# lesterphillip/SVCC23_FastSVC

Hardware: AMD Instinct MI355X
Metric: audio samples/sec (24 kHz) FastSVC generator fwd (higher is better)
Workload: dtype bf16 (bf16 MFMA products, f32 accumulate; bf16 storage); 1 GPU; cfg3: 64 x 10 s utterances per GPU, F=1500 frames, T=240000 samples, generator fastsvc.yaml (144->[192,96,48,24], x[2,4,4,5]), spk_emb on; global_batch=64, utterance_samples=240000, parallelism=utterance-parallel x1

## Files before the change

### include/fastsvc_hip.h

```cpp
#ifndef FASTSVC_HIP_H
#define FASTSVC_HIP_H

#include <stddef.h>
#include <stdint.h>

#ifdef __cplusplus
extern "C" {
#endif

#define FASTSVC_ABI_VERSION 1
#define FASTSVC_MAX_STAGES 8

enum {
    FASTSVC_OK = 0,
    FASTSVC_E_INVALID = -1,
    FASTSVC_E_MISSING = -2,
    FASTSVC_E_WORKSPACE = -3,
    FASTSVC_E_HIP = -4,
    FASTSVC_E_UNSUPPORTED = -5
};

typedef struct fastsvc_config {
    int32_t in_channels;
    int32_t n_stages;
// ... 46 lines not shown
                            float* out, int32_t B, int32_t F, const int32_t* lengths,
                            const int32_t* group, const int32_t* own_lo, const int32_t* own_hi,
                            void* workspace, size_t workspace_bytes,
                            void* scratch, size_t scratch_bytes, void* stream);

int fastsvc_norm_group_stats(const void* u, int32_t storage, int32_t B, int32_t C, int32_t ld, const int32_t* lengths,
                             int32_t len_mul, const int32_t* group, const int32_t* own_lo, const int32_t* own_hi,
                             double* stats_out, void* scratch, size_t scratch_bytes, void* stream);

int fastsvc_stream_prepare(void* stream);

int fastsvc_stream_release(void* stream);

void fastsvc_split_half(const float* x, int64_t n, uint16_t* f16_hi, uint16_t* f16_lo, uint16_t* bf16);

int fastsvc_workspace_tap(const fastsvc_plan* plan, int32_t B, int32_t F, const char* tap_name,
                          size_t* byte_offset, int64_t* numel, int64_t shape3[3]);

int fastsvc_autotune(const fastsvc_plan* plan, const void* dev_blob,
                     const float* ppg, const float* sine, const float* lft, const float* spk_emb,
                     float* out, int32_t B, int32_t F,
                     void* workspace, size_t workspace_bytes, void* stream, int32_t* n_trials);

int fastsvc_tuned_count(const fastsvc_plan* plan);
int fastsvc_tuned_get(const fastsvc_plan* plan, int32_t index, char* key_out, int32_t shape_out[5]);
int fastsvc_tuned_set(const fastsvc_plan* plan, const char* key, const int32_t shape[5]);

typedef struct fastsvc_launch_record {
    char layer[64];
    char kernel[40];
    double flops;
    double bytes;
    float ms;
} fastsvc_launch_record;

int fastsvc_forward_profile(const fastsvc_plan* plan, const void* dev_blob,
                            const float* ppg, const float* sine, const float* lft, const float* spk_emb,
                            float* out, int32_t B, int32_t F, const int32_t* lengths,
                            void* workspace, size_t workspace_bytes, void* stream,
                            fastsvc_launch_record* records, int32_t max_records, int32_t* n_records);

int fastsvc_forward_launch_count(const fastsvc_plan* plan, int32_t with_spk_emb);
double fastsvc_flops_per_sample(const fastsvc_plan* plan);

size_t fastsvc_signal_scratch_bytes(int32_t B, int32_t F);
int fastsvc_signal_generate(const float* f0, float* out, void* scratch, int32_t B, int32_t F, int32_t hop,
                            float sample_rate, float sine_amp, float noise_amp,
                            const int32_t* types, int32_t ntypes, uint64_t seed, void* stream);

int fastsvc_gather_padded(const float* const* src, const int32_t* lens, const int32_t* pitches, float* dst,
                          int32_t B, int32_t C, int32_t width, void* stream);

int fastsvc_gather_time_major(const float* packed, int64_t packed_elems, const int64_t* offsets, const int32_t* lens,
                              float* dst, int32_t B, int32_t C, int32_t width, void* stream);

int fastsvc_pcm16_pack(const float* y, const int32_t* lens, const int64_t* offsets, int16_t* dst, int64_t dst_elems,
                       int32_t B, int32_t width, void* stream);

typedef struct fastsvc_row_report {
    int32_t nonfinite;
    int32_t clipped;
    float   max_abs;
    int32_t reserved;
} fastsvc_row_report;

int fastsvc_pcm16_pack_checked(const float* y, const int32_t* lens, const int64_t* offsets, int16_t* dst, int64_t dst_elems,
// ... 80 lines not shown
```

### svcc23_fastsvc_amd/csrc/fastsvc_hx.hip

```cpp
#include "fastsvc_kernels.h"

namespace fastsvc {
#ifdef FASTSVC_ACT_2B
namespace FASTSVC_ACT_NS {
#endif

#include "fastsvc_device.inc"

#include "fastsvc_hx_common.inc"

template <int MW, int NW, bool RELOAD, bool OPT_LAST = false, int NS = 3 * MW * HX_NP, int SOFF = 0, bool ADV = true, bool HOLD = false>
__device__ __forceinline__ void hx_unit_direct(f32x4 (&acc)[NW][MW], const unsigned char* tile, const int (&aoff)[3],
                                               int lo_off, HxWeightStream<NS>& ws, bool do_last = true, bool hold = false) {
    constexpr int NSTEP = 3 * NW;
    constexpr int PF = HX_NP == 1 ? (MW >= 3 ? 2 : 3) : 1;
    HxFrag a[PF + 1];
    #pragma unroll
    for (int q = 0; q < PF && q < NSTEP; ++q) a[q] = hx_read(tile, aoff[q / NW] + (q % NW) * 16 * HX_ROW, lo_off);
    #pragma unroll
    for (int s = 0; s < NSTEP; ++s) {
        const int tap = s / NW, n = s % NW;
        if (s + PF < NSTEP) {
            a[(s + PF) % (PF + 1)] = hx_read(tile, aoff[(s + PF) / NW] + ((s + PF) % NW) * 16 * HX_ROW, lo_off);
            __builtin_amdgcn_sched_barrier(0);
// ... 426 lines not shown
    const __amdgpu_buffer_rsrc_t yr = make_rsrc(p.last_y + (long)b * p.last_y_b, p.ldy);
    #pragma unroll
    for (int n = 0; n < NW; ++n) {
        f32x4 s = acc[n][0] * kw[0];
        #pragma unroll
        for (int m = 1; m < MW; ++m) s += acc[n][m] * kw[m];
        #pragma unroll
        for (int e = 0; e < 4; ++e) {
            float v = s[e];
            v += __builtin_bit_cast(float, __builtin_amdgcn_mov_dpp(__builtin_bit_cast(int, v), 0xB1, 0xF, 0xF, true));
            v += __builtin_bit_cast(float, __builtin_amdgcn_mov_dpp(__builtin_bit_cast(int, v), 0x4E, 0xF, 0xF, true));
            v += __builtin_bit_cast(float, __builtin_amdgcn_mov_dpp(__builtin_bit_cast(int, v), 0x141, 0xF, 0xF, true));
            v += __builtin_bit_cast(float, __builtin_amdgcn_mov_dpp(__builtin_bit_cast(int, v), 0x140, 0xF, 0xF, true));
            s[e] = v;
        }
        const int t = PAIRS ? tcol0 + (n >> 1) * 32 + (lane >> 4) * 8 + (n & 1) * 4 : tcol0 + n * 16 + (lane >> 4) * 4;
        buf_store4(yr, ((lane & 15) == 0 && t < p.T) ? t * 4 : OOB_OFF, s + bias);
    }
}

#ifndef FASTSVC_HX_W8
#define FASTSVC_HX_W8 1
#endif
constexpr bool hx_w8(int MODE, bool tailk, int S) {
    return FASTSVC_HX_W8 != 0 && HX_NP == 1 && !tailk && (MODE == MODE_DIRECT || MODE == MODE_POLY || (MODE == MODE_DEC2 && S == 2));
}
#ifndef FASTSVC_HX_CARRY
#define FASTSVC_HX_CARRY 1
#endif
constexpr bool hx_carry(int MODE, bool tailk, int S, int NT) {
    return FASTSVC_HX_CARRY != 0 && hx_w8(MODE, tailk, S) && MODE == MODE_DIRECT && S == 1 && NT == 128;
}

template <int MW, int NW, int WM, int WN, int MODE, int EPI, int S, bool WSTATIC, bool TAILK = false>
__global__ __launch_bounds__(512, (hx_min_waves<MW, NW, MODE, EPI, S, TAILK>()))
void conv_hx_kernel(const ConvParams p0) {
    constexpr bool UPH = MODE == MODE_UPHEAD;
    constexpr bool POLY = MODE == MODE_POLY, DEC2 = MODE == MODE_DEC2, CHAIN = MODE == MODE_CHAIN || MODE == MODE_CHAIN1 || UPH;
    constexpr bool IN1 = MODE == MODE_CHAIN1;
    constexpr bool WLB = MODE == MODE_CHAIN && S == 2;
    constexpr bool XR = MODE == MODE_DIRECT && S > 1;
    constexpr int NT = 16 * NW * WN;
    constexpr int NTV = CHAIN ? NT + 16 : NT;
    constexpr int HB = CHAIN ? 4 : 0;
    constexpr int NPROD_T = 256;
    constexpr bool W8 = hx_w8(MODE, TAILK, S);
    constexpr int SPARE = W8 ? 8 : 4;
    constexpr int MAXW = NTV + (MODE == MODE_DIRECT ? (W8 ? 64 : 56) : (W8 ? 16 : 8));
    constexpr int ITEMS = (MAXW + NPROD_T - 1) / NPROD_T;
    constexpr int NWS = DEC2 ? 4 : 3;
    constexpr int NVAR = DEC2 ? 2 : 1;
    constexpr int NSLOT = NWS * MW * HX_NP;
    constexpr bool TRACKS = AMAX_TRACK && ((CHAIN && MODE != MODE_UPHEAD) || (MODE == MODE_DIRECT && (EPI == EPI_RES || EPI == EPI_RANK1)));
    extern __shared__ __attribute__((aligned(16))) unsigned char smem_raw[];

    const int tid = threadIdx.x;
    const int lane = tid & 63;
    const int wave = __builtin_amdgcn_readfirstlane(tid >> 6);
    const bool producer = wave >= 4;
    const int cw = wave & 3;
    const int wave_m = cw / WN;
    const int wave_n = cw - wave_m * WN;
    const int z = blockIdx.z;
    const int sig = z / p0.B;
    const int b = z - sig * p0.B;
    ConvParams p = p0;
    if (p0.lens) {
        const int frames = p0.lens[b];
        p.T = frames * p0.len_mul;
        p.x_T = frames * p0.xlen_mul;
    }
    const int mg = blockIdx.y * WM + wave_m;
    const bool active = !producer && mg < p.ngroups;
    const int halo = (MODE == MODE_DIRECT || CHAIN) ? p.dil : 1;
// ... 1 lines not shown
    const int W = NTV + 2 * halo_al;
    const int nch = p.nch32;
    const int CINp = nch * HX_KC;
    const int flags = p.flags;
    const int ntx = (p.T + NT - 1) / NT;
    const int tile0 = blockIdx.x * p.tpw;
    const int ntiles = min(p.tpw, ntx - tile0);
    if (ntiles <= 0) return;
    const int nunits = ntiles * (XR ? 2 * nch : nch);
#ifdef FASTSVC_TIMELINE
    const int wg_lin = blockIdx.x + gridDim.x * (blockIdx.y + gridDim.y * blockIdx.z);
    unsigned long long* tlw = (p.tl && wg_lin < p.tl_wgs) ? p.tl + ((long)wg_lin * 8 + wave) * 64 : nullptr;
    int tli = 0;
    auto stamp = [&](int tag) {
        if (tlw && lane == 0 && tli < 62) { tlw[tli++] = ((unsigned long long)tag << 56) | (__builtin_readcyclecounter() & 0x00ffffffffffffffull); }
    };
    stamp(1);
    if (tlw && lane == 0) {
        tlw[62] = __builtin_amdgcn_s_getreg(4 | (0 << 6) | (31 << 11));
        tlw[63] = __builtin_amdgcn_s_getreg(20 | (0 << 6) | (31 << 11));
    }
#else
    auto stamp = [](int) {};
#endif

    if constexpr (hx_min_waves<MW, NW, MODE, EPI, S, TAILK>() >= 4) {
        const int wg_id = blockIdx.x + gridDim.x * (blockIdx.y + gridDim.y * blockIdx.z);
        if ((wg_id >> 8) & 1) {
            for (int k = 0; k < p.stagger; ++k) __builtin_amdgcn_s_sleep(16);
        }
    }
    double* sstat = reinterpret_cast<double*>(smem_raw);
    float2* ncoef = reinterpret_cast<float2*>(smem_raw + sizeof(double) * 2 * 16 * MW * WM);
    unsigned char* tiles = reinterpret_cast<unsigned char*>(ncoef + CINp + 8);
    __shared__ unsigned s_amax, s_cnt;
    __shared__ float s_inv[HX_NP == 2 ? 2 * 16 * MW * WM : 4];
    __shared__ __attribute__((aligned(16))) float s_mid[CHAIN ? 2 * (16 * MW * WM + 32) : 4];
    float sx = 1.f;
    float sx2 = 1.f;
    float s_mid_scale = 1.f;
    const int ninv = 16 * MW * p.ngroups;
    const float* invtab = (HX_NP == 2 && p.whx_inv) ? p.whx_inv + (long)sig * p.whx_inv_sig : nullptr;
    auto operand_scales = [&]() {
#ifndef FASTSVC_EXP_NOSCALE
        if constexpr (HX_NP == 2) {
            if (p.amax_in) {
                auto bound_of = [&](int entry, int s) -> float {
                    float bd = amax_read(p.amax_in, entry);
                    #pragma unroll
                    for (int j = 0; j < 2; ++j)
                        if (p.bnd_path[j]) { const float* q = p.bnd_path[j] + (long)s * p.bnd_sig[j]; bd = bd * q[0] + q[1]; }
                    return bd;
                };
                float bound = bound_of(sig * p.amax_in_sig + b, sig);
                if (p.amax_in2 > 0) bound = fmaxf(bound, bound_of(p.amax_in2 + b, 1));
                if (flags & F_PRE_NORM) bound += sqrtf((float)p.x_T);
                if constexpr (CHAIN) {
                    if (invtab) {
                        const float* cst = invtab + (UPH ? 3 : 2) * ninv;
                        if constexpr (IN1) bound = bound * cst[2] + cst[3];
                        s_mid_scale = hx_scale_for(bound * cst[0] + cst[1]);
                    }
                }
                sx = hx_scale_for(bound);
            }
            if constexpr (XR) {
                if (p.amax_x2) {
// ... 347 lines not shown
            if constexpr (XR) {
                const int tl = xc_tl;
                pos_next(xc_tl, xc_ch);
                const int t_start = (tile0 + tl) * NT - halo_al;
                const int g0 = (t_start + 8 * XROWS) / XROWS - 8;
                const int r0 = (g0 + xg) * XROWS - t_start;
                #pragma unroll
                for (int jj = 0; jj < XJ; ++jj) {
                    float px[XJ][8];
                    #pragma unroll
                    for (int c = 0; c < 8; ++c) px[jj][c] = act_unpack1(pw[jj][c]);
                    hx8 h;
                    #pragma unroll
                    for (int c = 0; c < 8; ++c) h[c] = (hx_t)(HX_NP == 2 ? px[jj][c] * sx2 : px[jj][c]);
                    typedef unsigned u32x4w __attribute__((ext_vector_type(4)));
                    u32x4w lp = {0u, 0u, 0u, 0u};
                    if constexpr (HX_NP == 2) {
                        const u32x4w hp = __builtin_bit_cast(u32x4w, h);
                        #pragma unroll
                        for (int k = 0; k < 4; ++k) lp[k] = hx_lo_pair(hp[k], px[jj][2 * k] * sx2, px[jj][2 * k + 1] * sx2);
                    }
                    #pragma unroll
                    for (int ph = 0; ph < S; ++ph) {
                        const int r = r0 + jj * S + ph;
                        const int off = hx_lds_off((unsigned)r < (unsigned)W ? r : W, xoct);
                        *reinterpret_cast<hx8*>(tile + off) = h;
                        if constexpr (HX_NP == 2) *reinterpret_cast<u32x4w*>(tile + lo_off + off) = lp;
                    }
                }
            }
        };
        if constexpr (XR) {
            pwin_t pa[ITEMS][8];
            act1_t xb[XJ][8];
            unsigned oka = 0;
            pload(0, pa, oka);
            ploadX(1, xb);
            stamp(2);
            setup_shared();
            pcommit(0, pa, oka, tiles);
            unsigned okn = 0;
            if constexpr (!WSTATIC) pload(2, pa, okn);
            stamp(3);
            __syncthreads();
            stamp(4);
            for (int u = 0; u < nunits; u += 2) {
                if constexpr (WSTATIC) pload(u + 2, pa, oka);
                pcommitX(u + 1, xb, tiles + bufsz);
                if constexpr (!WSTATIC) ploadX(u + 3, xb);
                stamp(5);
                __syncthreads();
                stamp(6);
                if constexpr (WSTATIC) ploadX(u + 3, xb); else oka = okn;
                pcommit(u + 2, pa, oka, tiles);
                if constexpr (!WSTATIC) pload(u + 4, pa, okn);
                stamp(5);
                __syncthreads();
                stamp(6);
            }
        } else {
        constexpr bool PSPLIT = POLY && hx_poly_staged<MW, NW, MODE, EPI, S>();
        EpiRsrc Rp;
        const bool pact = mg < p.ngroups;
        if constexpr (PSPLIT) {
            const long ct = (long)p.COUT * p.ldy;
            const float* nul = p.bias;
            Rp.y = act_rsrc(p.y ? p.y : nul, p.y ? (long)sig * p.y_sig + (long)b * p.y_b : 0, p.y ? ct : 0);
            const bool has_y2 = (flags & F_AFF_OUT) != 0;
            Rp.y2 = act_rsrc(has_y2 ? p.y2 : nul, has_y2 ? (long)sig * p.y2_sig + (long)b * p.y2_b : 0, has_y2 ? ct : 0);
            const bool has_ss = (flags & (F_STATS | F_AFF_OUT)) != 0;
            Rp.ss = act_rsrc(has_ss ? p.ss_out : nul, has_ss ? (long)b * p.ss_out_b : 0, has_ss ? 2 * ct : 0);
            Rp.res = Rp.y; Rp.r1x = Rp.y;
        }
        auto ppass2 = [&](int un) {
#ifdef FASTSVC_ACT_2B
            if constexpr (PSPLIT) {
                const int etl = e_tl, ech = e_ch;
                pos_next(e_tl, e_ch);
                if (un < nunits && ech == nch - 1) {
                    const int tcolw = (tile0 + etl) * NT + wave_n * (NW * 16);
                    const unsigned char* Pw = tiles + 2 * bufsz + cw * hx_poly_patch_bytes<MW, NW, S>();
                    HxPolyPass2<MW, NW, EPI, S, hx_poly_mc<MW>(), MW> P2;
                    float s1p[MW], s2p[MW];
                    #pragma unroll
                    for (int m = 0; m < MW; ++m) { s1p[m] = 0.f; s2p[m] = 0.f; }
                    if (pact) P2.request(p, Rp, mg, tcolw, lane);
                    __syncthreads();
                    if (pact) {
                        P2.run(p, Rp, Pw, s1p, s2p, mg, tcolw, lane);
                        if (flags & F_STATS) {
                            #pragma unroll
// ... 718 lines not shown
        }
#define FASTSVC_HXC(k) if (kind == k) return hx_launch_kind<MW, NW, WM, WN, MODE_CHAIN, k, 1>(grid, smem, stream, p);
        FASTSVC_HXC(EPI_PLAIN) FASTSVC_HXC(EPI_RES) FASTSVC_HXC(EPI_RANK1)
#undef FASTSVC_HXC
        return hipErrorInvalidValue;
    } else if constexpr (MODE == MODE_DEC2) {
        const size_t patch = hx_dec2_staged<MW, NW, MODE_DEC2>() ? 4 * (size_t)hx_dec2_patch_bytes<MW, NW>() : 0;
        if (p.s == 1 && (p.ldx & 3) == 0) return hx_launch_kind<MW, NW, WM, WN, MODE_DEC2, EPI_PLAIN, 2>(grid, smem + patch, stream, p);
        return hx_launch_kind<MW, NW, WM, WN, MODE_DEC2, EPI_PLAIN, 1>(grid, smem + patch, stream, p);
    } else if constexpr (MODE == MODE_POLY) {
#define FASTSVC_HXP(sv) \
        if (p.s == sv) return aff ? hx_launch_kind<MW, NW, WM, WN, MODE_POLY, EPI_AFF, sv>(grid, smem + (hx_poly_staged<MW, NW, MODE_POLY, EPI_AFF, sv>() ? 4 * hx_poly_patch_bytes<MW, NW, sv>() : 0), stream, p) \
                                  : hx_launch_kind<MW, NW, WM, WN, MODE_POLY, EPI_PLAIN, sv>(grid, smem + (hx_poly_staged<MW, NW, MODE_POLY, EPI_PLAIN, sv>() ? 4 * hx_poly_patch_bytes<MW, NW, sv>() : 0), stream, p);
        FASTSVC_HXP(2) FASTSVC_HXP(4) FASTSVC_HXP(5)
#undef FASTSVC_HXP
        return hipErrorInvalidValue;
    } else {
        const int kind = aff ? EPI_AFF : p.r1x ? EPI_RANK1 : p.res ? EPI_RES : EPI_PLAIN;
        size_t est = 0;
        constexpr bool PAIRS = hx_pairs_epi<MW, NW, MODE_DIRECT>();
        if ((kind == EPI_AFF && hx_estage<MW, NW, MODE_DIRECT, EPI_AFF>()) || (kind == EPI_RES && hx_estage<MW, NW, MODE_DIRECT, EPI_RES>()))
            est = sizeof(float) * 4 * (size_t)(aff ? (p.res ? 3 : 2) : 1) * (PAIRS ? MW * (NW / 2) * 256 : MW * NW * EST_ITEM_FLOATS);
        if (MW == 2 && p.nch32 == 1 && !p.x2 &&
            ((kind == EPI_AFF && hx_est2<MW, NW, MODE_DIRECT, EPI_AFF>()) || (kind == EPI_RES && hx_est2<MW, NW, MODE_DIRECT, EPI_RES>())))
            est *= 2;
        if (PAIRS) est += sizeof(float) * 4 * 16 * 36;
        if (kind == EPI_AFF && hx_two_cu<MW, NW, MODE_DIRECT, EPI_AFF>() && !(p.lens && (((p.len_mul | p.xlen_mul) & 3) != 0)))
            est += hx_gsum_bytes<MW>();
        if (p.x2) {
            if (kind != EPI_AFF || p.res || p.x2_T * p.s2 != p.T || (p.lens && (((p.len_mul | p.xlen_mul) & 3) != 0)))
                return hipErrorInvalidValue;
            if (w8 && p.s2 == 2 && W / p.s2 + 5 > 128) return hipErrorInvalidValue;
            if (w8 && !conv_hx_x2_rows_ok(p)) return hipErrorInvalidValue;
#define FASTSVC_HXX(sv, stat) if (p.s2 == sv) return hx_launch_instance<&conv_hx_kernel<MW, NW, WM, WN, MODE_DIRECT, EPI_AFF, sv, stat>>(grid, smem + est, stream, p);
            if constexpr (MW * NW <= 12) {
                if constexpr (MW == 2) { if (p.nch32 == 1) { FASTSVC_HXX(5, true) } }
                else { FASTSVC_HXX(2, false) FASTSVC_HXX(4, false) }
            }
#undef FASTSVC_HXX
            return hipErrorInvalidValue;
        }
#define FASTSVC_HX(k) if (kind == k) return hx_launch_kind<MW, NW, WM, WN, MODE_DIRECT, k, 1>(grid, smem + est, stream, p);
        FASTSVC_HX(EPI_PLAIN) FASTSVC_HX(EPI_RES) FASTSVC_HX(EPI_RANK1) FASTSVC_HX(EPI_AFF)
#undef FASTSVC_HX
        return hipErrorInvalidValue;
    }
}

hipError_t launch_conv_hx(const ConvParams& p, const ConvLaunch& cfg, hipStream_t stream) {
    if (p.ntaps != 3 || (p.T & 3) || !p.whx || p.nch32 * HX_KC > 512) return hipErrorInvalidValue;
#define FASTSVC_HXS(md, mw, nw, wm, wn) \
    if (cfg.MW == mw && cfg.NW == nw && cfg.WM == wm && cfg.WN == wn) \
        return hx_launch_shape<mw, nw, wm, wn, md>(p, cfg.nsig, stream);
    if (p.mode == MODE_DIRECT) {
        if (p.dil < 1 || p.dil > 28) return hipErrorInvalidValue;
        FASTSVC_HXS(MODE_DIRECT, 2, 2, 1, 4) FASTSVC_HXS(MODE_DIRECT, 2, 3, 1, 4)
        FASTSVC_HXS(MODE_DIRECT, 3, 2, 1, 4) FASTSVC_HXS(MODE_DIRECT, 3, 3, 1, 4)
        FASTSVC_HXS(MODE_DIRECT, 3, 4, 2, 2) FASTSVC_HXS(MODE_DIRECT, 3, 6, 2, 2)
        FASTSVC_HXS(MODE_DIRECT, 3, 8, 4, 1)
    } else if (p.mode == MODE_POLY) {
        if (p.dil != 1) return hipErrorInvalidValue;
        FASTSVC_HXS(MODE_POLY, 2, 2, 1, 4) FASTSVC_HXS(MODE_POLY, 2, 3, 1, 4)
        FASTSVC_HXS(MODE_POLY, 3, 2, 1, 4) FASTSVC_HXS(MODE_POLY, 3, 2, 2, 2)
    } else if (p.mode == MODE_CHAIN) {
        if (p.dil < 1 || p.dil > 4 || p.dil2 < 1 || p.dil2 > 4 || !p.bias_mid || p.CMID != p.COUT) return hipErrorInvalidValue;
        if (p.ngroups > cfg.WM) return hipErrorInvalidValue;
        FASTSVC_HXS(MODE_CHAIN, 2, 2, 1, 4) FASTSVC_HXS(MODE_CHAIN, 2, 3, 1, 4)
        FASTSVC_HXS(MODE_CHAIN, 3, 2, 1, 4) FASTSVC_HXS(MODE_CHAIN, 3, 3, 1, 4)
        FASTSVC_HXS(MODE_CHAIN, 3, 4, 2, 2) FASTSVC_HXS(MODE_CHAIN, 3, 6, 2, 2)
    } else if (p.mode == MODE_UPHEAD) {
        if (p.dil != 1 || p.dil2 != 1 || !p.bias_mid || p.CMID != p.COUT || p.ngroups > cfg.WM) return hipErrorInvalidValue;
        FASTSVC_HXS(MODE_UPHEAD, 3, 4, 4, 1) FASTSVC_HXS(MODE_UPHEAD, 3, 2, 2, 2)
        FASTSVC_HXS(MODE_UPHEAD, 3, 2, 1, 4) FASTSVC_HXS(MODE_UPHEAD, 2, 2, 1, 4)
    } else if (p.mode == MODE_CHAIN1) {
        if (p.dil < 1 || p.dil > 4 || p.dil2 < 1 || p.dil2 > 4 || !p.bias_mid || p.CMID != p.COUT || p.CIN > 32 ||
            !p.in1_w || !p.in1_b || p.ngroups > cfg.WM) return hipErrorInvalidValue;
        FASTSVC_HXS(MODE_CHAIN1, 2, 2, 1, 4) FASTSVC_HXS(MODE_CHAIN1, 2, 3, 1, 4)
    } else if (p.mode == MODE_DEC2) {
        if (p.dil != 1 || !p.bias2 || !p.y2) return hipErrorInvalidValue;
        FASTSVC_HXS(MODE_DEC2, 3, 2, 1, 4) FASTSVC_HXS(MODE_DEC2, 3, 3, 1, 4) FASTSVC_HXS(MODE_DEC2, 3, 2, 2, 2)
        FASTSVC_HXS(MODE_DEC2, 3, 4, 2, 2) FASTSVC_HXS(MODE_DEC2, 3, 4, 4, 1)
    }
#undef FASTSVC_HXS
    return hipErrorInvalidValue;
}

#ifndef FASTSVC_ACT_2B
bool conv_hx_x2_ok(int MW, int nch32, int s2) { return MW == 2 ? (nch32 == 1 && s2 == 5) : MW == 3 ? (s2 == 2 || s2 == 4) : false; }
bool conv_hx_x2_rows_ok(const ConvParams& p) { return p.s2 != 2 || ((p.lens ? p.x2len_mul : p.x2_T) & 3) == 0; }
bool conv_hx_tail_ok(int mode, int MW, int epi_kind, int S) { return hx_tail_instance(MW, mode, epi_kind, S); }

bool conv_hx_shape(int mode, int MW, int NW, int WM, int WN) {
    if (mode == MODE_POLY)
        return (MW == 2 && WM == 1 && WN == 4 && (NW == 2 || NW == 3)) ||
               (MW == 3 && NW == 2 && ((WM == 1 && WN == 4) || (WM == 2 && WN == 2)));
    if (mode == MODE_DEC2)
        return MW == 3 && ((WM == 1 && WN == 4 && (NW == 2 || NW == 3)) || (WM == 2 && WN == 2 && (NW == 2 || NW == 4)) ||
                           (WM == 4 && WN == 1 && NW == 4));
    if (mode == MODE_CHAIN1) return MW == 2 && WM == 1 && WN == 4 && (NW == 2 || NW == 3);
    if (mode == MODE_UPHEAD)
        return (MW == 3 && ((NW == 4 && WM == 4 && WN == 1) || (NW == 2 && WM == 2 && WN == 2) || (NW == 2 && WM == 1 && WN == 4))) ||
               (MW == 2 && NW == 2 && WM == 1 && WN == 4);
    if (mode == MODE_CHAIN)
        return (WM == 1 && WN == 4 && (MW == 2 || MW == 3) && (NW == 2 || NW == 3)) ||
               (MW == 3 && WM == 2 && WN == 2 && (NW == 4 || NW == 6));
    if (mode != MODE_DIRECT) return false;
    if (MW == 2) return WM == 1 && WN == 4 && (NW == 2 || NW == 3);
    if (MW != 3) return false;
    if (WM == 1 && WN == 4) return NW == 2 || NW == 3;
    if (WM == 2 && WN == 2) return NW == 4 || NW == 6;
    return WM == 4 && WN == 1 && NW == 8;
}
#endif

#ifdef FASTSVC_ACT_2B
}
#endif
}
```

### svcc23_fastsvc_amd/csrc/fastsvc_kernels.h

```cpp
#pragma once
#include <hip/hip_runtime.h>
#include <stdint.h>

#if defined(FASTSVC_ACT_BF16) && defined(FASTSVC_ACT_F16)
#error "FASTSVC_ACT_BF16 and FASTSVC_ACT_F16 exclude each other"
#endif
#if defined(FASTSVC_ACT_BF16)
#define FASTSVC_ACT_2B 1
#define FASTSVC_ACT_NS bf16
#elif defined(FASTSVC_ACT_F16)
#define FASTSVC_ACT_2B 1
#define FASTSVC_ACT_NS f16
#endif

namespace fastsvc {

enum : int {
    MODE_DIRECT = 0,
    MODE_DECIMATE = 1,
    MODE_STRETCH = 2,
    MODE_POLY = 3,
    MODE_WINO = 4,
    MODE_DEC2 = 5,
    MODE_CHAIN = 6,
    MODE_CHAIN1 = 7,
    MODE_UPHEAD = 8
};

enum : int {
    F_PRE_LRELU = 1,
    F_PRE_AFFINE = 2,
    F_PRE_NORM = 4,
    F_POST_LRELU = 8,
    F_STATS = 16,
    F_AFF_OUT = 32
};

constexpr float LRELU_SLOPE = 0.2f;
constexpr double IN_EPS = 1e-5;

struct ConvParams {
    const float* x;
    long x_sig, x_b;
    int x_T;
    int CIN, KC, nchunks;
    const float* w;
    long w_sig;
    const float* bias;
    long bias_sig;
    int Q;
    const void* whx;
    long whx_sig;
    int nch32;
    int stagger;
    const float* bias_mid;
    long bias_mid_sig;
    const float* last_w;
    const float* last_b;
    float* last_y;
    long last_y_b;
    int xsplit;
    const float* in1_w;
    const float* in1_b;
    long in1_w_sig, in1_b_sig;
    int CMID, nch32b, dil2;
    int ngroups;
    const float* whx_inv;
    long whx_inv_sig;
// ... 103 lines not shown
    long hd_sig, hd_b;
    int hd_ld, hd_s;
    int tpw;
    int small;
};

enum : int { DBG_NO_LOAD = 1, DBG_NO_MFMA = 2, DBG_NO_EPILOGUE = 4, DBG_NO_COMMIT = 8, DBG_NO_WEIGHTS = 16 };
#ifdef FASTSVC_DEBUG_SWITCHES
#define FASTSVC_DBG_ON(p, flag) (((p).dbg & (flag)) != 0)
#else
#define FASTSVC_DBG_ON(p, flag) false
#endif

struct ConvLaunch {
    int MW;
    int NW;
    int WM, WN;
    int nsig;
    int pipe;
};

bool conv_pipe_supported(const ConvParams& p);
bool conv_poly_shape(int MW, int NW, int WM, int WN);
int conv_ws_resident(int MW, int NW, int mode, int epi_kind);
bool conv_ws_tail_ok(int MW, int NW, int mode, int epi_kind, int S);

hipError_t launch_conv(const ConvParams& p, const ConvLaunch& cfg, hipStream_t stream);

hipError_t launch_conv_hx(const ConvParams& p, const ConvLaunch& cfg, hipStream_t stream);
bool conv_hx_shape(int mode, int MW, int NW, int WM, int WN);
bool conv_hx_tail_ok(int mode, int MW, int epi_kind, int S);
bool conv_hx_x2_ok(int MW, int nch32, int s2);
bool conv_hx_x2_rows_ok(const ConvParams& p);

hipError_t launch_conv_wx(const ConvParams& p, const ConvLaunch& cfg, hipStream_t stream);
bool conv_wx_shape(int mode, int MW, int NW, int WM, int WN);
bool conv_wx_fits(int nch32, int dil);
bool conv_wx_supported(const ConvParams& p);

hipError_t launch_in1_conv(const float* x, long x_sig, const float* w, const float* bias, long w_sig, long b_sig,
                           float* y, int nsig, int B, int C, int T, const int* lens, int len_mul, hipStream_t stream,
                           float* amax_out = nullptr);

hipError_t launch_noop(hipStream_t stream);
hipError_t launch_stats_exact(const float* u, double* st, int B, int C, int ld, const int* lens, int len_mul, int max_frames,
                              hipStream_t stream);
hipError_t launch_amax_inputs(const float* sig, long sig_stride, const float* ppg, int B, int C, int F, int hop,
                              const int* lens, float* amax_in, float* zero, int nzero, hipStream_t stream);

constexpr int NORMGROUP_CHUNK = 2048;
inline int norm_group_chunks(long ld) { return (int)((ld + NORMGROUP_CHUNK - 1) / NORMGROUP_CHUNK); }
hipError_t launch_norm_group_partials(const float* u, double* part, int B, int C, int ld, const int* lens, int len_mul,
                                      const int* group, const int* own_lo, const int* own_hi, hipStream_t stream);
hipError_t launch_norm_group_pool(const double* part, double* st, int B, int C, int ld, const int* lens, int len_mul,
                                  const int* group, const int* own_lo, const int* own_hi, float* amax_raise, hipStream_t stream);

hipError_t launch_pointwise_out(const float* x, const float* w, const float* bias, float* y,
                                int B, int C, int O, int T, const int* lens, int len_mul, hipStream_t stream);

hipError_t launch_cond_stage0(const CondStage0Params& p, hipStream_t stream);
int cond_stage0_tile_columns(int small);
hipError_t launch_cond_stage1(const CondStage1Params& p, hipStream_t stream);
int cond_stage1_tile_columns(int small);

struct SpkBlock {
    const float* w;
// ... 29 lines not shown
```

### svcc23_fastsvc_amd/csrc/fastsvc_plan.cpp

```cpp
#include <hip/hip_runtime.h>

#include <algorithm>
#include <chrono>
#include <cmath>
#include <cstddef>
#include <cstdio>
#include <cstdlib>
#include <cstring>
#include <functional>
#include <map>
#include <mutex>
#include <thread>
#include <type_traits>
#include <atomic>
#include <string>
#include <unordered_map>
#include <vector>

#include "fastsvc_hip.h"
#include "fastsvc_kernels.h"
#include "fastsvc_pack.h"

using namespace fastsvc;

// ... 1675 lines not shown
    auto it = tuned.find(key);
    const size_t n = std::strlen(key);
    if (it == tuned.end() && n >= 2 && key[n - 2] == '|' && key[n - 1] == 'h') {
        std::string kb(key);
        kb[n - 1] = 'b';
        it = tuned.find(kb);
    }
    return it;
}
inline const char* prod_tag(int storage) { return storage == 2 ? "h1" : storage == 1 ? "x1" : "x3"; }
#define FASTSVC_BY_STORAGE(storage, fn) ((storage) == 2 ? f16::fn : (storage) == 1 ? bf16::fn : fn)
void print_choice(const char* layer, const char* kernel, int tpw, int small = -1) {
    if (!env().verbose_shapes) return;
    if (small >= 0) std::fprintf(stderr, "[fastsvc] %s %s tpw %d small %d\n", layer, kernel, tpw, small);
    else std::fprintf(stderr, "[fastsvc] %s %s tpw %d\n", layer, kernel, tpw);
}


bool table_entry(const fastsvc_plan& P, const char* key, fastsvc_plan::Choice& out) {
    std::lock_guard<std::mutex> lock(P.tune_mu);
    auto it = tuned_find(P.tuned, key);
    if (it == P.tuned.end()) return false;
    out = it->second;
    return true;
}
void table_record(const fastsvc_plan& P, const char* key, const fastsvc_plan::Choice& ch) {
    std::lock_guard<std::mutex> lock(P.tune_mu);
    P.tuned[key] = ch;
    P.priors.clear();
}

struct Cand { int NW, WM, WN, algo; };

struct EventPair {
    hipEvent_t e0 = nullptr, e1 = nullptr;
    ~EventPair() { if (e0) hipEventDestroy(e0); if (e1) hipEventDestroy(e1); }
    bool create() { return hipEventCreate(&e0) == hipSuccess && hipEventCreate(&e1) == hipSuccess; }
};

template <class PrepareFn, class LaunchFn>
hipError_t time_candidates(const std::vector<Cand>& cands, hipStream_t stream, int& trials, PrepareFn&& prepare, LaunchFn&& launch,
                           Cand& best, int& best_tpw, float& best_ms) {
    static const int tpws[] = {1, 2, 3, 4, 5, 6, 7, 8, 9, 10, 11, 12, 14, 16, 20, 24};
    EventPair ev;
    if (!ev.create()) return hipErrorUnknown;
    best_ms = 1e30f;
    for (const Cand& cd : cands) {
        const long ntx = prepare(cd);
        for (int tpw : tpws) {
            hipError_t e = launch(tpw);
            if (e != hipSuccess && cd.algo == 6) break;
            if (e != hipSuccess) return e;
            hipEventRecord(ev.e0, stream);
            for (int r = 0; r < 3; ++r) { e = launch(tpw); if (e != hipSuccess) return e; }
            hipEventRecord(ev.e1, stream);
            if (hipEventSynchronize(ev.e1) != hipSuccess) return hipErrorUnknown;
            float ms = 0.f;
            hipEventElapsedTime(&ms, ev.e0, ev.e1);
            ++trials;
            if (ms < best_ms) { best_ms = ms; best = cd; best_tpw = tpw; }
            if (tpw >= ntx) break;
        }
    }
    return hipSuccess;
}

// ... 188 lines not shown
                   int what, double sep_ms, bool& done) {
    done = false;
    const PackedConv& c = u.d3;
    const int stg = cc.storage;
    const bool act_2b = stg != 0;
    const int prec = stg;
    p.ldx = p.x_T; p.ldy = p.T; p.ldx2 = p.x2_T;
    if (p.lens) { p.len_mul = p.T / p.frames_ld; p.xlen_mul = p.x_T / p.frames_ld; p.x2len_mul = p.x2_T / p.frames_ld; }
    if (!env().hx || !env().d3x || cc.exact_f32 || p.no_hx || !c.hxc_off[prec] || (p.T & 3) || p.x_T != p.T || (long)p.x2_T * p.s2 != p.T ||
        (p.lens && (((p.len_mul | p.xlen_mul) & 3) != 0)) || !conv_hx_x2_ok(c.MW, c.nch32, p.s2) || c.dil > 28 ||
        (act_2b && !conv_hx_x2_rows_ok(p)))
        return hipSuccess;
    p.mode = MODE_DIRECT; p.s = 1;
    p.CIN = c.cin; p.KC = c.KC; p.nchunks = c.nchunks; p.w = blob + c.w_off; p.Q = c.Q;
    p.COUT = c.cout; p.ngroups = c.ngroups; p.ntaps = 3; p.dil = c.dil; p.nch32 = c.nch32;
    p.whx = blob + c.hxc_off[prec]; p.whx_sig = 0;
    p.whx_inv = prec == 0 ? blob + c.hxc_inv_off : nullptr; p.whx_inv_sig = 0;
    p.bias = blob + c.b_off; p.bias_sig = 0; p.bias2 = blob + c.b2_off; p.bias2_sig = 0;
    p.res = nullptr;
    p.vec = 1; p.tpw = 1; p.xs = 0; p.ps = 0;
    p.stagger = env().stagger; p.dbg = env().dbg;
    auto launch = [&](const ConvParams& q, const ConvLaunch& Lq) {
        return FASTSVC_BY_STORAGE(stg, launch_conv_hx)(q, Lq, stream);
    };
    std::vector<Cand> cands;
    static const int shapes[][3] = {{4, 2, 2}, {2, 1, 4}, {3, 1, 4}, {2, 2, 2}};
    for (const auto& sh : shapes)
        if (conv_hx_shape(MODE_DIRECT, c.MW, sh[0], sh[1], sh[2]) && c.ngroups % sh[1] == 0 && sh[0] * c.MW <= 12)
            cands.push_back(Cand{sh[0], sh[1], sh[2], 3});
    if (cands.empty()) return hipSuccess;
    char key[96];
    std::snprintf(key, sizeof(key), "%s|%d|%d%s", layer, p.B, p.T, key_suffix(stg));
    bool have = false, fused = true;
    Cand best = cands[0];
    fastsvc_plan::Choice ch;
    if (table_entry(*cc.plan, key, ch)) {
        if (ch.algo != 3 && env().d3x != 2) { have = true; fused = false; }
        for (const Cand& cd : cands)
            if (cd.NW == ch.NW && cd.WM == ch.WM && cd.WN == ch.WN && ch.tpw >= 1 && ch.tpw <= 64) { best = cd; p.tpw = ch.tpw; have = true; }
    }
    auto ntx_of = [&](const Cand& cd) { return (long)(p.T + 16 * cd.NW * cd.WN - 1) / (16 * cd.NW * cd.WN); };
    if (what == 2) {
        if (have || !cc.tuning) return hipSuccess;
        float best_ms = 1e30f;
        ConvParams q = p;
        q.flags &= ~F_STATS;
        ConvLaunch Lq{c.MW, 0, 0, 0, 1, 2};
        hipError_t e = time_candidates(cands, stream, cc.trials,
                                       [&](const Cand& cd) { Lq.NW = cd.NW; Lq.WM = cd.WM; Lq.WN = cd.WN; return ntx_of(cd); },
                                       [&](int tpw) { q.tpw = tpw; return launch(q, Lq); }, best, p.tpw, best_ms);
        if (e != hipSuccess) return e;
        fused = sep_ms <= 0.0 || best_ms / 3.0 < sep_ms;
        table_record(*cc.plan, key, fastsvc_plan::Choice{best.NW, best.WM, best.WN, p.tpw, fused ? 3 : 0});
        return hipSuccess;
    }
    if (!have) {
        if (cc.tuning) return hipSuccess;
        {
            fastsvc_plan::Choice pr{0, 0, 0, 0, -1};
            std::lock_guard<std::mutex> lock(cc.plan->tune_mu);
            if (cc.plan->prior_for(layer, p.B, p.T, act_2b, pr)) {
                if (pr.algo != 3 && env().d3x != 2) fused = false;
                for (const Cand& cd : cands) if (cd.NW == pr.NW && cd.WM == pr.WM && cd.WN == pr.WN) best = cd;
            }
        }
        p.tpw = fill_tpw(ntx_of(best), (long)(c.ngroups / best.WM) * p.B, c.nch32, 24);
    }
    if (!fused) return hipSuccess;
    done = true;
    if (what == 0) return hipSuccess;
    ConvLaunch L{c.MW, best.NW, best.WM, best.WN, 1, 2};
    double flops = 0.0, bytes = 0.0;
    char kname[48] = "";
    if (prof) {
        const double cols = (double)p.T * p.B;
        flops = 2.0 * 2.0 * 3.0 * c.cin * c.cout * cols;
        const double el = (double)c.cin * p.T + (double)c.cin * p.x2_T + 4.0 * c.cout * p.T;
        bytes = (act_2b ? 2.0 : 4.0) * el * p.B + 4.0 * 2.0 * (double)(c.w_floats + c.b_floats);
        std::snprintf(kname, sizeof(kname), "conv_hx<%d,%d,%d,%d,0,4,%d,%s>", L.MW, L.NW, L.WM, L.WN, p.s2, prod_tag(stg));
    }
    const long wgs = ((ntx_of(best) + p.tpw - 1) / p.tpw) * (long)(c.ngroups / L.WM) * p.B;
    return launch_tail(prof, stream, layer, kname, p.tpw, -1, flops, bytes, [&]() { return launch(p, L); }, &p, &L, wgs, 2 * p.nch32);
}

hipError_t run_cond_stage0(const CallCtx& cc, const float* blob, const float* sig, long sig_stride, int B, long T, int F,
                           const int* lengths, float* ss, float* hd, const float* amax_in, float* amax_hd, hipStream_t stream,
                           Profiler* prof, bool& done) {
    done = false;
    const fastsvc_plan& P = *cc.plan;
    if (!cond_stage_whole(P, 0, F) || cc.exact_f32 || (P.storage == 0 && (!amax_in || !amax_hd))) return hipSuccess;
    const DownStage& d = P.down[0];
    const DownStage& d1 = P.down[1];
    const int prec = P.storage;
    CondStage0Params q;
    std::memset(&q, 0, sizeof(q));
    q.x = sig; q.x_sig = sig_stride; q.x_b = T;
    q.B = B; q.C = d.C; q.T = (int)T; q.ld = (int)T;
    q.lens = lengths; q.len_mul = (int)(T / F);
    const PackedConv* layers[3] = {d.c2, d.c3, d.film};
    for (int s = 0; s < 2; ++s) {
        q.in1_w[s] = blob + d.c1_raw[s].w_off; q.in1_b[s] = blob + d.c1_raw[s].b_off;
        q.r1w[s] = blob + d.r_raw[s].w_off; q.r1b[s] = blob + d.r_raw[s].b_off;
        for (int l = 0; l < 3; ++l) {
            q.w[l][s] = blob + layers[l][s].hx_off[prec];
            q.bias[l][s] = blob + layers[l][s].b_off;
            q.winv[l][s] = blob + layers[l][s].hx_inv_off;
            q.bnd[l + 1][s] = blob + layers[l][s].bnd_off;
        }
        q.bnd[0][s] = blob + d.c1_raw[s].bnd_off;
        q.bnd_r[s] = blob + d.r_raw[s].bnd_off;
        q.cbnd[s] = d.cbnd_off[s] ? blob + d.cbnd_off[s] : nullptr;
    }
    q.w5 = blob + d.heads.hx_off[prec]; q.b5 = blob + d.heads.b_off; q.winv5 = blob + d.heads.hx_inv_off;
    q.amax_in = P.storage == 0 ? amax_in : nullptr; q.amax_hd = P.storage == 0 ? amax_hd : nullptr;
    q.ss = ss; q.ss_b = 2L * d.C * T;
// ... 1115 lines not shown
```

### svcc23_fastsvc_amd/engine.py

```python
from __future__ import annotations

import ctypes
import json
import os
from typing import Dict, Mapping, Optional, Sequence, Tuple

import numpy as np
import torch

from .synth import GeneratorConfig

_LIB = None
_LIB_PATH = os.environ.get("FASTSVC_HIP_LIB") or \
    os.path.join(os.path.dirname(os.path.abspath(__file__)), "libfastsvc_hip.so")
MAX_STAGES = 8
STORAGE_CODES = {"float32": 0, "bfloat16": 1, "float16": 2}
STORAGE_DTYPES = {"float32": torch.float32, "bfloat16": torch.bfloat16, "float16": torch.float16}
TUNED_TABLE_PATH = os.path.join(os.path.dirname(os.path.abspath(__file__)), "tuned_mi355x.json")

ABI_SYMBOLS = (
    "fastsvc_abi_version", "fastsvc_last_error", "fastsvc_plan_create", "fastsvc_plan_destroy",
    "fastsvc_plan_set_storage", "fastsvc_plan_get_storage",
    "fastsvc_weight_blob_bytes", "fastsvc_pack_weights", "fastsvc_workspace_bytes",
    "fastsvc_pack_device_scratch_bytes", "fastsvc_pack_device_launch_count", "fastsvc_pack_weights_device",
# ... 3 lines not shown
    "fastsvc_stream_prepare", "fastsvc_stream_release", "fastsvc_split_half", "fastsvc_plan_set_workspace_mode",
    "fastsvc_loudness_frames", "fastsvc_loudness_scratch_bytes", "fastsvc_loudness_extract",
    "fastsvc_gather_padded", "fastsvc_gather_time_major", "fastsvc_pcm16_pack",
    "fastsvc_pcm16_pack_checked", "fastsvc_output_check",
    "fastsvc_collate_launch_count", "fastsvc_collate_crops",
    "fastsvc_fanout_launch_count", "fastsvc_fanout_assemble",
    "fastsvc_window_launch_count", "fastsvc_window_assemble", "fastsvc_window_stitch",
    "fastsvc_stft_loss_scratch_bytes", "fastsvc_stft_loss_forward", "fastsvc_stft_loss_backward",
    "fastsvc_conv1d_forward", "fastsvc_conv1d_backward_weight", "fastsvc_conv1d_backward_weight_scratch_bytes",
    "fastsvc_film_norm_forward", "fastsvc_film_norm_backward", "fastsvc_weight_norm_forward", "fastsvc_weight_norm_backward",
    "fastsvc_gconv1d_supported", "fastsvc_gconv1d_forward", "fastsvc_gconv1d_backward_data",
    "fastsvc_gconv1d_backward_weight_scratch_bytes", "fastsvc_gconv1d_backward_weight",
)


class FastSVCError(RuntimeError):
    pass


class _Config(ctypes.Structure):
    _fields_ = [
        ("in_channels", ctypes.c_int32),
        ("n_stages", ctypes.c_int32),
        ("mid_channels", ctypes.c_int32 * MAX_STAGES),
        ("upsampling_scales", ctypes.c_int32 * MAX_STAGES),
        ("out_channels", ctypes.c_int32),
        ("spk_emb_size", ctypes.c_int32),
        ("use_spk_emb", ctypes.c_int32),
    ]


class _LaunchRecord(ctypes.Structure):
    _fields_ = [("layer", ctypes.c_char * 64), ("kernel", ctypes.c_char * 40),
                ("flops", ctypes.c_double), ("bytes", ctypes.c_double), ("ms", ctypes.c_float)]


class _Tensor(ctypes.Structure):
    _fields_ = [("name", ctypes.c_char_p), ("data", ctypes.POINTER(ctypes.c_float)), ("numel", ctypes.c_int64)]


def library_path() -> str:
    return _LIB_PATH


def load_library():
    global _LIB
    if _LIB is not None:
        return _LIB
    if not os.path.exists(_LIB_PATH):
        raise FastSVCError(
            f"{_LIB_PATH} not found: build it with `python -m svcc23_fastsvc_amd.build` "
            "(hipcc --offload-arch=gfx950). There is no CPU fallback for this path.")
    lib = ctypes.CDLL(_LIB_PATH)
    vp, sz, i32, i64 = ctypes.c_void_p, ctypes.c_size_t, ctypes.c_int32, ctypes.c_int64
    lib.fastsvc_abi_version.restype = ctypes.c_int
    lib.fastsvc_last_error.restype = ctypes.c_char_p
    lib.fastsvc_plan_create.argtypes = [ctypes.POINTER(_Config), ctypes.POINTER(vp)]
    lib.fastsvc_plan_create.restype = ctypes.c_int
    lib.fastsvc_plan_destroy.argtypes = [vp]
    lib.fastsvc_plan_destroy.restype = None
    lib.fastsvc_plan_set_storage.argtypes = [vp, i32]
    lib.fastsvc_plan_set_storage.restype = ctypes.c_int
    lib.fastsvc_plan_get_storage.argtypes = [vp]
    lib.fastsvc_plan_get_storage.restype = ctypes.c_int
    lib.fastsvc_weight_blob_bytes.argtypes = [vp]
    lib.fastsvc_weight_blob_bytes.restype = sz
    lib.fastsvc_pack_weights.argtypes = [vp, ctypes.POINTER(_Tensor), i32, vp]
# ... 902 lines not shown
            raise ValueError(f"out must be a contiguous float32 {(B, cfg.out_channels, T)} tensor on {dev}")
        with torch.cuda.device(dev):
            stream = torch.cuda.current_stream(dev).cuda_stream
            common = (
                self._h, ctypes.c_void_p(blob.data_ptr()),
                ctypes.c_void_p(ppg.data_ptr()), ctypes.c_void_p(sine.data_ptr()),
                ctypes.c_void_p(lft.data_ptr()),
                ctypes.c_void_p(spk_emb.data_ptr()) if spk_emb is not None else None,
                ctypes.c_void_p(out.data_ptr()), B, F,
                ctypes.c_void_p(lens_dev.data_ptr()) if lens_dev is not None else None,
                ctypes.c_void_p(workspace.data_ptr()), workspace.numel(), ctypes.c_void_p(stream))
            if autotune:
                ntr = ctypes.c_int32(0)
                rc = self.lib.fastsvc_autotune(*common[:9], common[10], common[11], common[12], ctypes.byref(ntr))
                self.last_autotune_trials = int(ntr.value)
            elif norm_groups is not None and spk_emb is not None:
                need = self.norm_group_scratch_bytes(B, F)
                if norm_scratch is None or norm_scratch.numel() * norm_scratch.element_size() < need or norm_scratch.device != dev:
                    norm_scratch = torch.empty(need, dtype=torch.uint8, device=dev)
                ng = self._stage_lengths(torch.tensor(norm_groups, dtype=torch.int32).reshape(-1), 3 * B, dev)
                rc = self.lib.fastsvc_forward_grouped(*common[:10], *[ctypes.c_void_p(ng[i * B:].data_ptr()) for i in range(3)],
                                                      common[10], common[11], ctypes.c_void_p(norm_scratch.data_ptr()),
                                                      norm_scratch.numel() * norm_scratch.element_size(), common[12])
                workspace = (workspace, ng, norm_scratch)
            elif profile is None:
                rc = self.lib.fastsvc_forward(*common)
            else:
                recs = (_LaunchRecord * 256)()
                n = ctypes.c_int32(0)
                rc = self.lib.fastsvc_forward_profile(*common, recs, 256, ctypes.byref(n))
                if rc == 0:
                    for i in range(n.value):
                        profile.append(dict(layer=recs[i].layer.decode(), kernel=recs[i].kernel.decode(),
                                            flops=recs[i].flops, bytes=recs[i].bytes, ms=recs[i].ms))
        _check(self.lib, rc, "fastsvc_forward")
        self._last_workspace = (workspace, lens_dev)
        return out
```

Before: 1.821 billion samples/s.

## Stage strided x2 input via coalesced 128-bit gather into LDS for S=4/5

```diff
diff --git a/include/fastsvc_hip.h b/include/fastsvc_hip.h
--- a/include/fastsvc_hip.h
+++ b/include/fastsvc_hip.h
@@ -102,6 +102,7 @@
     double flops;
     double bytes;
     float ms;
+    int32_t x2_path;
 } fastsvc_launch_record;
 
 int fastsvc_forward_profile(const fastsvc_plan* plan, const void* dev_blob,
diff --git a/svcc23_fastsvc_amd/csrc/fastsvc_hx.hip b/svcc23_fastsvc_amd/csrc/fastsvc_hx.hip
--- a/svcc23_fastsvc_amd/csrc/fastsvc_hx.hip
+++ b/svcc23_fastsvc_amd/csrc/fastsvc_hx.hip
@@ -482,6 +482,18 @@
     return FASTSVC_HX_CARRY != 0 && hx_w8(MODE, tailk, S) && MODE == MODE_DIRECT && S == 1 && NT == 128;
 }
 
+constexpr int HX_X2G_COLS = 64;
+constexpr int HX_X2G_ROW = HX_X2G_COLS * 2;
+constexpr int HX_X2G_GROUP = 8 * HX_X2G_ROW + 32;
+constexpr int HX_X2G_BYTES = 4 * HX_X2G_GROUP;
+constexpr bool hx_x2_gather(int MODE, int S) {
+#ifdef FASTSVC_ACT_2B
+    return MODE == MODE_DIRECT && (S == 4 || S == 5);
+#else
+    return false;
+#endif
+}
+
 template <int MW, int NW, int WM, int WN, int MODE, int EPI, int S, bool WSTATIC, bool TAILK = false>
 __global__ __launch_bounds__(512, (hx_min_waves<MW, NW, MODE, EPI, S, TAILK>()))
 void conv_hx_kernel(const ConvParams p0) {
@@ -490,6 +502,7 @@
     constexpr bool IN1 = MODE == MODE_CHAIN1;
     constexpr bool WLB = MODE == MODE_CHAIN && S == 2;
     constexpr bool XR = MODE == MODE_DIRECT && S > 1;
+    constexpr bool XG = XR && hx_x2_gather(MODE, S);
     constexpr int NT = 16 * NW * WN;
     constexpr int NTV = CHAIN ? NT + 16 : NT;
     constexpr int HB = CHAIN ? 4 : 0;
@@ -557,7 +570,8 @@
     }
     double* sstat = reinterpret_cast<double*>(smem_raw);
     float2* ncoef = reinterpret_cast<float2*>(smem_raw + sizeof(double) * 2 * 16 * MW * WM);
-    unsigned char* tiles = reinterpret_cast<unsigned char*>(ncoef + CINp + 8);
+    unsigned char* x2raw = reinterpret_cast<unsigned char*>(ncoef + CINp + 8);
+    unsigned char* tiles = x2raw + ((XG && (p0.flags & F_X2_GATHER)) ? HX_X2G_BYTES : 0);
     __shared__ unsigned s_amax, s_cnt;
     __shared__ float s_inv[HX_NP == 2 ? 2 * 16 * MW * WM : 4];
     __shared__ __attribute__((aligned(16))) float s_mid[CHAIN ? 2 * (16 * MW * WM + 32) : 4];
@@ -971,8 +985,83 @@
         };
         if constexpr (XR) {
             pwin_t pa[ITEMS][8];
+            unsigned oka = 0;
+            bool gathered = false;
+#ifdef FASTSVC_ACT_2B
+            if constexpr (XG) {
+                gathered = (flags & F_X2_GATHER) != 0;
+                if (gathered) {
+                    typedef unsigned u32x4w __attribute__((ext_vector_type(4)));
+                    const int g_rr = ptid >> 3, g_pc = ptid & 7;
+                    const int g_dst = (g_rr >> 3) * HX_X2G_GROUP + (g_rr & 7) * HX_X2G_ROW + g_pc * 16;
+                    auto gloadX = [&](int un, u32x4w& w, int& nv) {
+                        const int tl = xl_tl, ch = xl_ch;
+                        pos_next(xl_tl, xl_ch);
+                        const int t_start = (tile0 + tl) * NT - halo_al;
+                        const int g0 = (t_start + 8 * S) / S - 8;
+                        const int jc = (g0 & ~7) + 8 * g_pc;
+                        const bool ok = ((unsigned)jc < (unsigned)x2T) & (g_rr < p.CIN - ch * HX_KC) & (un < nunits);
+                        nv = ok ? min(8, x2T - jc) : 0;
+                        w = __builtin_amdgcn_raw_buffer_load_b128(x2r, ok ? (g_rr * p.ldx2 + jc) * 2 : OOB_OFF, ch * HX_KC * p.ldx2 * 2, FASTSVC_LD_AUX);
+                    };
+                    auto gstoreX = [&](const u32x4w& w, int nv) {
+                        u32x4w v = w;
+                        asm volatile("" : "+v"(v));
+                        #pragma unroll
+                        for (int k = 0; k < 4; ++k) v[k] &= nv >= 2 * k + 2 ? 0xffffffffu : nv == 2 * k + 1 ? 0x0000ffffu : 0u;
+                        *reinterpret_cast<u32x4w*>(x2raw + g_dst) = v;
+                        __builtin_amdgcn_sched_barrier(0);
+                    };
+                    auto gcommitX = [&](unsigned char* tile) {
+                        const int tl = xc_tl;
+                        pos_next(xc_tl, xc_ch);
+                        const int t_start = (tile0 + tl) * NT - halo_al;
+                        const int g0 = (t_start + 8 * S) / S - 8;
+                        const int r0 = (g0 + xg) * S - t_start;
+                        const unsigned char* src = x2raw + xoct * HX_X2G_GROUP + min((g0 & 7) + xg, HX_X2G_COLS - 1) * 2;
+                        hx8 h;
+                        #pragma unroll
+                        for (int c = 0; c < 8; ++c)
+                            h[c] = (hx_t)act_unpack1((act1_t)*reinterpret_cast<const unsigned short*>(src + c * HX_X2G_ROW));
+                        #pragma unroll
+                        for (int ph = 0; ph < S; ++ph) {
+                            const int r = r0 + ph;
+                            *reinterpret_cast<hx8*>(tile + hx_lds_off((unsigned)r < (unsigned)W ? r : W, xoct)) = h;
+                        }
+                    };
+                    u32x4w xw;
+                    int xn = 0;
+                    unsigned okn = 0;
+                    pload(0, pa, oka);
+                    gloadX(1, xw, xn);
+                    stamp(2);
+                    setup_shared();
+                    pcommit(0, pa, oka, tiles);
+                    gstoreX(xw, xn);
+                    if constexpr (!WSTATIC) pload(2, pa, okn);
+                    stamp(3);
+                    __syncthreads();
+                    stamp(4);
+                    for (int u = 0; u < nunits; u += 2) {
+                        if constexpr (WSTATIC) pload(u + 2, pa, oka);
+                        gcommitX(tiles + bufsz);
+                        if constexpr (!WSTATIC) gloadX(u + 3, xw, xn);
+                        stamp(5);
+                        __syncthreads();
+                        stamp(6);
+                        if constexpr (WSTATIC) gloadX(u + 3, xw, xn); else oka = okn;
+                        pcommit(u + 2, pa, oka, tiles);
+                        gstoreX(xw, xn);
+                        if constexpr (!WSTATIC) pload(u + 4, pa, okn);
+                        stamp(5);
+                        __syncthreads();
+                        stamp(6);
+                    }
+                }
+            }
+#endif
+            if (!gathered) {
             act1_t xb[XJ][8];
-            unsigned oka = 0;
             pload(0, pa, oka);
             ploadX(1, xb);
             stamp(2);
@@ -996,6 +1085,7 @@
                 stamp(5);
                 __syncthreads();
                 stamp(6);
+            }
             }
         } else {
         constexpr bool PSPLIT = POLY && hx_poly_staged<MW, NW, MODE, EPI, S>();
@@ -1780,6 +1870,10 @@
                 return hipErrorInvalidValue;
             if (w8 && p.s2 == 2 && W / p.s2 + 5 > 128) return hipErrorInvalidValue;
             if (w8 && !conv_hx_x2_rows_ok(p)) return hipErrorInvalidValue;
+            if (p.flags & F_X2_GATHER) {
+                if (!hx_x2_gather(MODE_DIRECT, p.s2) || !conv_hx_x2_gather_ok(p, NT)) return hipErrorInvalidValue;
+                est += HX_X2G_BYTES;
+            }
 #define FASTSVC_HXX(sv, stat) if (p.s2 == sv) return hx_launch_instance<&conv_hx_kernel<MW, NW, WM, WN, MODE_DIRECT, EPI_AFF, sv, stat>>(grid, smem + est, stream, p);
             if constexpr (MW * NW <= 12) {
                 if constexpr (MW == 2) { if (p.nch32 == 1) { FASTSVC_HXX(5, true) } }
@@ -1836,6 +1930,11 @@
 #ifndef FASTSVC_ACT_2B
 bool conv_hx_x2_ok(int MW, int nch32, int s2) { return MW == 2 ? (nch32 == 1 && s2 == 5) : MW == 3 ? (s2 == 2 || s2 == 4) : false; }
 bool conv_hx_x2_rows_ok(const ConvParams& p) { return p.s2 != 2 || ((p.lens ? p.x2len_mul : p.x2_T) & 3) == 0; }
+bool conv_hx_x2_gather_ok(const ConvParams& p, int NT) {
+    const int W = NT + 2 * ((p.dil + 7) & ~7);
+    return (p.s2 == 4 || p.s2 == 5) && (p.ldx2 & 7) == 0 && (p.x2_b & 7) == 0 && (reinterpret_cast<uintptr_t>(p.x2) & 15) == 0 &&
+           W <= (HX_X2G_COLS - 8) * p.s2 + 1;
+}
 bool conv_hx_tail_ok(int mode, int MW, int epi_kind, int S) { return hx_tail_instance(MW, mode, epi_kind, S); }
 
 bool conv_hx_shape(int mode, int MW, int NW, int WM, int WN) {
diff --git a/svcc23_fastsvc_amd/csrc/fastsvc_kernels.h b/svcc23_fastsvc_amd/csrc/fastsvc_kernels.h
--- a/svcc23_fastsvc_amd/csrc/fastsvc_kernels.h
+++ b/svcc23_fastsvc_amd/csrc/fastsvc_kernels.h
@@ -33,7 +33,8 @@
     F_PRE_NORM = 4,
     F_POST_LRELU = 8,
     F_STATS = 16,
-    F_AFF_OUT = 32
+    F_AFF_OUT = 32,
+    F_X2_GATHER = 64
 };
 
 constexpr float LRELU_SLOPE = 0.2f;
@@ -203,6 +204,7 @@
 bool conv_hx_tail_ok(int mode, int MW, int epi_kind, int S);
 bool conv_hx_x2_ok(int MW, int nch32, int s2);
 bool conv_hx_x2_rows_ok(const ConvParams& p);
+bool conv_hx_x2_gather_ok(const ConvParams& p, int NT);
 
 hipError_t launch_conv_wx(const ConvParams& p, const ConvLaunch& cfg, hipStream_t stream);
 bool conv_wx_shape(int mode, int MW, int NW, int WM, int WN);
diff --git a/svcc23_fastsvc_amd/csrc/fastsvc_plan.cpp b/svcc23_fastsvc_amd/csrc/fastsvc_plan.cpp
--- a/svcc23_fastsvc_amd/csrc/fastsvc_plan.cpp
+++ b/svcc23_fastsvc_amd/csrc/fastsvc_plan.cpp
@@ -1731,6 +1731,9 @@
 
 struct Cand { int NW, WM, WN, algo; };
 
+inline bool d3x_fused_algo(int algo) { return algo == 3 || algo == 7 || algo == 8; }
+inline bool d3x_gather_default(int s2) { return s2 == 4 || s2 == 5; }
+
 struct EventPair {
     hipEvent_t e0 = nullptr, e1 = nullptr;
     ~EventPair() { if (e0) hipEventDestroy(e0); if (e1) hipEventDestroy(e1); }
@@ -1985,14 +1988,19 @@
     char key[96];
     std::snprintf(key, sizeof(key), "%s|%d|%d%s", layer, p.B, p.T, key_suffix(stg));
     bool have = false, fused = true;
+    int x2_path = 3;
     Cand best = cands[0];
     fastsvc_plan::Choice ch;
     if (table_entry(*cc.plan, key, ch)) {
-        if (ch.algo != 3 && env().d3x != 2) { have = true; fused = false; }
+        if (d3x_fused_algo(ch.algo)) x2_path = ch.algo;
+        else if (env().d3x != 2) { have = true; fused = false; }
         for (const Cand& cd : cands)
             if (cd.NW == ch.NW && cd.WM == ch.WM && cd.WN == ch.WN && ch.tpw >= 1 && ch.tpw <= 64) { best = cd; p.tpw = ch.tpw; have = true; }
     }
     auto ntx_of = [&](const Cand& cd) { return (long)(p.T + 16 * cd.NW * cd.WN - 1) / (16 * cd.NW * cd.WN); };
+    auto gather_for = [&](const Cand& cd) {
+        return (act_2b && x2_path != 7 && (x2_path == 8 || d3x_gather_default(p.s2)) && conv_hx_x2_gather_ok(p, 16 * cd.NW * cd.WN)) ? (int)F_X2_GATHER : 0;
+    };
     if (what == 2) {
         if (have || !cc.tuning) return hipSuccess;
         float best_ms = 1e30f;
@@ -2000,7 +2008,7 @@
         q.flags &= ~F_STATS;
         ConvLaunch Lq{c.MW, 0, 0, 0, 1, 2};
         hipError_t e = time_candidates(cands, stream, cc.trials,
-                                       [&](const Cand& cd) { Lq.NW = cd.NW; Lq.WM = cd.WM; Lq.WN = cd.WN; return ntx_of(cd); },
+                                       [&](const Cand& cd) { Lq.NW = cd.NW; Lq.WM = cd.WM; Lq.WN = cd.WN; q.flags = (q.flags & ~F_X2_GATHER) | gather_for(cd); return ntx_of(cd); },
                                        [&](int tpw) { q.tpw = tpw; return launch(q, Lq); }, best, p.tpw, best_ms);
         if (e != hipSuccess) return e;
         fused = sep_ms <= 0.0 || best_ms / 3.0 < sep_ms;
@@ -2013,7 +2021,8 @@
             fastsvc_plan::Choice pr{0, 0, 0, 0, -1};
             std::lock_guard<std::mutex> lock(cc.plan->tune_mu);
             if (cc.plan->prior_for(layer, p.B, p.T, act_2b, pr)) {
-                if (pr.algo != 3 && env().d3x != 2) fused = false;
+                if (d3x_fused_algo(pr.algo)) x2_path = pr.algo;
+                else if (env().d3x != 2) fused = false;
                 for (const Cand& cd : cands) if (cd.NW == pr.NW && cd.WM == pr.WM && cd.WN == pr.WN) best = cd;
             }
         }
@@ -2023,6 +2032,7 @@
     done = true;
     if (what == 0) return hipSuccess;
     ConvLaunch L{c.MW, best.NW, best.WM, best.WN, 1, 2};
+    p.flags = (p.flags & ~F_X2_GATHER) | gather_for(best);
     double flops = 0.0, bytes = 0.0;
     char kname[48] = "";
     if (prof) {
@@ -2033,7 +2043,10 @@
         std::snprintf(kname, sizeof(kname), "conv_hx<%d,%d,%d,%d,0,4,%d,%s>", L.MW, L.NW, L.WM, L.WN, p.s2, prod_tag(stg));
     }
     const long wgs = ((ntx_of(best) + p.tpw - 1) / p.tpw) * (long)(c.ngroups / L.WM) * p.B;
-    return launch_tail(prof, stream, layer, kname, p.tpw, -1, flops, bytes, [&]() { return launch(p, L); }, &p, &L, wgs, 2 * p.nch32);
+    return launch_tail(prof, stream, layer, kname, p.tpw, -1, flops, bytes, [&]() {
+        if (prof && act_2b && (p.s2 == 4 || p.s2 == 5)) prof->recs.back().x2_path = (p.flags & F_X2_GATHER) ? 2 : 1;
+        return launch(p, L);
+    }, &p, &L, wgs, 2 * p.nch32);
 }
 
 hipError_t run_cond_stage0(const CallCtx& cc, const float* blob, const float* sig, long sig_stride, int B, long T, int F,
diff --git a/svcc23_fastsvc_amd/engine.py b/svcc23_fastsvc_amd/engine.py
--- a/svcc23_fastsvc_amd/engine.py
+++ b/svcc23_fastsvc_amd/engine.py
@@ -59,7 +59,7 @@
 
 class _LaunchRecord(ctypes.Structure):
     _fields_ = [("layer", ctypes.c_char * 64), ("kernel", ctypes.c_char * 40),
-                ("flops", ctypes.c_double), ("bytes", ctypes.c_double), ("ms", ctypes.c_float)]
+                ("flops", ctypes.c_double), ("bytes", ctypes.c_double), ("ms", ctypes.c_float), ("x2_path", ctypes.c_int32)]
 
 
 class _Tensor(ctypes.Structure):
@@ -1028,7 +1028,8 @@
                 if rc == 0:
                     for i in range(n.value):
                         profile.append(dict(layer=recs[i].layer.decode(), kernel=recs[i].kernel.decode(),
-                                            flops=recs[i].flops, bytes=recs[i].bytes, ms=recs[i].ms))
+                                            flops=recs[i].flops, bytes=recs[i].bytes, ms=recs[i].ms,
+                                            x2_path=("", "element", "gather")[recs[i].x2_path]))
         _check(self.lib, rc, "fastsvc_forward")
         self._last_workspace = (workspace, lens_dev)
         return out
```

Result: faster. 1.839 billion samples/s, median of 6 (+1.0%).
